# creanero/MKIDS_SDR

Hardware: AMD Instinct MI355X
Metric: ADC MSample/s/GPU at 1024 ch; achieved HBM GB/s vs roofline (higher is better)
Workload: dtype int16 in, fp32 DSP, int16 Fix16_13 trigger

## Files before the change

mkids_sdr_amd/csrc/k_trigger.hip:

```cpp
#include <algorithm>
#include <type_traits>

#include "mkid_plan.h"
#include "trig_common.h"

namespace mkid {

constexpr int kSpecThreads = 256;
constexpr int32_t kFullWarm = 100;

__device__ __forceinline__ int64_t seg_state(const TrigSpecArgs& a, int c, int s) { return (int64_t)c * a.nseg + s; }
__device__ __forceinline__ int64_t seg_begin(const TrigSpecArgs& a, int s) { return (int64_t)s * a.L; }
__device__ __forceinline__ int64_t seg_end(const TrigSpecArgs& a, int s) {
    return seg_begin(a, s) + a.L < a.J ? seg_begin(a, s) + a.L : a.J;
}
__device__ __forceinline__ int64_t slot_entry(const TrigSpecArgs& a, int c, int s) {
    return (int64_t)c * a.seg_stride + a.seg_base + s;
}
__device__ __forceinline__ TrigCfg trig_cfg(const TrigSpecArgs& a, int c) {
    return TrigCfg{a.thr[c], a.rearm[c], a.mode, a.alpha, a.kf, a.kq, a.base_thr, a.dead};
}

static_assert(plan::kSegL > kHoldOff + 1 && plan::kSvfLmin > kHoldOff + 1, "segments outlast the hold-off");

__device__ __forceinline__ int32_t raw_at(const TrigSpecArgs& a, int c, int64_t jj) {
    return jj >= 0 ? a.raw[jj * a.C + c] : (jj >= -kRawHist ? a.rhist[(jj + kRawHist) * a.C + c] : 0);
}

__device__ __attribute__((noinline)) uint64_t make_packet(int32_t c, EvInfo ev, int32_t f, int64_t jg) {
    return pack_wide(c, peakfit_i(ev.y1, ev.y2, f), ev.base, jg - 1);
}

struct Win {
    int32_t w[kFirTaps];
};

__device__ __forceinline__ void load_window(Win& win, const TrigSpecArgs& a, int c, int64_t j) {
    win.w[0] = 0;
#pragma unroll
    for (int i = 1; i < kFirTaps; ++i) win.w[i] = raw_at(a, c, j - kFirTaps + i);
}

__device__ __forceinline__ int32_t mf_at(const Win& win, const int32_t (&tap)[kFirTaps], int u) {
    int32_t acc = 0;
#pragma unroll
    for (int i = 0; i < kFirTaps; ++i) acc = __mul24(tap[i], win.w[(u - i + kFirTaps) % kFirTaps]) + acc;
    return mf_out(acc);
}

typedef short short2_t __attribute__((ext_vector_type(2)));
struct QWin {
    uint32_t q[kFirTaps];
    uint32_t last;
    uint32_t sel;
};

__device__ __forceinline__ uint32_t pack2(int32_t lo, int32_t hi) {
    return ((uint32_t)lo & 0xffffu) | ((uint32_t)hi << 16);
}

__device__ __forceinline__ short2_t as_s2(uint32_t v) { return __builtin_bit_cast(short2_t, v); }

__device__ __forceinline__ void load_tap_pairs(uint32_t (&tp)[kFirTaps / 2], const TrigSpecArgs& a, int c) {
#pragma unroll
    for (int m = 0; m < kFirTaps / 2; ++m) tp[m] = pack2(a.fir[c * kFirTaps + 2 * m], a.fir[c * kFirTaps + 2 * m + 1]);
}

__device__ __forceinline__ void load_qwin(QWin& w, const TrigSpecArgs& a, int c, int64_t j) {
    int32_t prev = 0;
#pragma unroll
    for (int i = 0; i < kFirTaps; ++i) {
        const int32_t r = raw_at(a, c, j - kFirTaps + i);
        w.q[i] = pack2(r, prev);
        prev = r;
    }
    w.last = pack2(prev, prev);
    w.sel = (c & 1) ? 0x07060302u : 0x05040100u;
}

struct Lim16 {
    int32_t lo, hi;
};
__device__ __forceinline__ Lim16 lim16() {
    Lim16 lim{-32768, 32767};
    asm volatile("" : "+v"(lim.lo), "+v"(lim.hi));
    return lim;
}
__device__ __forceinline__ int32_t mf_q(QWin& w, const uint32_t (&tp)[kFirTaps / 2], int u, uint32_t r,
                                        const Lim16& lim) {
    w.q[u] = __builtin_amdgcn_perm(w.last, r, w.sel);
    w.last = r;
    int32_t acc;
    asm("v_dot2_i32_i16 %0, %1, %2, 0" : "=v"(acc) : "v"(tp[0]), "v"(w.q[u]));
#pragma unroll
    for (int m = 1; m < kFirTaps / 2; ++m)
        acc = __builtin_amdgcn_sdot2(as_s2(tp[m]), as_s2(w.q[(u - 2 * m + 2 * kFirTaps) % kFirTaps]), acc, false);
    int32_t v;
    asm("v_med3_i32 %0, %1, %2, %3" : "=v"(v) : "v"(acc >> 11), "v"(lim.lo), "v"(lim.hi));
    return v;
}

__device__ __forceinline__ __amdgpu_buffer_rsrc_t raw_rsrc(const char* base) {
    return __builtin_amdgcn_make_buffer_rsrc(const_cast<char*>(base), (short)0, (int)0xffffffff, 0x00020000);
}

template <class F, class E>
__device__ __forceinline__ void run_groups(int32_t ngroups, const char* rbase, uint32_t& rrow, uint32_t lane,
                                           uint32_t row, F&& body, E&& half_end) {
    constexpr int H = kFirTaps / 2;
    const __amdgpu_buffer_rsrc_t rs = raw_rsrc(rbase);
    auto ld = [&](uint32_t off) { return (uint32_t)__builtin_amdgcn_raw_buffer_load_b32(rs, (int)lane, (int)off, 0); };
    auto uni = [](uint32_t v) { return (uint32_t)__builtin_amdgcn_readfirstlane((int)v); };
    uint32_t ra[H], rb[H];
    if (ngroups <= 0) return;
    rrow = uni(rrow);
#pragma unroll
    for (int u = 0; u < H; ++u) ra[u] = ld(rrow + (uint32_t)u * row);
    for (int32_t g = 0; g < ngroups; ++g) {
        const uint32_t cur = uni(rrow);
#pragma unroll
        for (int u = 0; u < H; ++u) rb[u] = ld(cur + (uint32_t)(H + u) * row);
#pragma unroll
        for (int u = 0; u < H; ++u) body(g, u, ra[u]);
        half_end(g, 0);
        const uint32_t nxt = uni(cur + (g + 1 < ngroups ? (uint32_t)kFirTaps * row : 0u));
#pragma unroll
        for (int u = 0; u < H; ++u) ra[u] = ld(nxt + (uint32_t)u * row);
#pragma unroll
        for (int u = 0; u < H; ++u) body(g, H + u, rb[u]);
        half_end(g, 1);
        rrow = cur + (uint32_t)kFirTaps * row;
    }
}
template <class F>
__device__ __forceinline__ void run_groups(int32_t ngroups, const char* rbase, uint32_t& rrow, uint32_t lane,
                                           uint32_t row, F&& body) {
    run_groups(ngroups, rbase, rrow, lane, row, body, [](int32_t, int) {});
}


template <int MODE, bool FAST = true>
struct Stepper {
    TrigState st;
    TrigCfg k;
    __device__ Stepper(const TrigState& s, const TrigCfg& kk) : st(s), k(kk) {}
    __device__ __forceinline__ bool step(int32_t f, EvInfo& ev) { return trig_update(st, f, k, ev); }
    __device__ __forceinline__ TrigState state() const { return st; }
};

template <int MODE>
struct Stepper<MODE, true> {
    FastState fs;
    FastCfg q;
    __device__ Stepper(const TrigState& s, const TrigCfg& k, int32_t f0) : fs(to_fast(s)), q(fast_cfg(k)) {
        if (!s.binit) fs.B = MODE == MKID_BASE_NONE ? 0 : f0;
    }
    __device__ __forceinline__ bool step(int32_t f, EvInfo& ev) { return trig_update_fast<MODE>(fs, f, q, ev); }
    __device__ __forceinline__ TrigState state() const { return from_fast(fs); }
};

template <>
struct Stepper<MKID_BASE_SVF, true> {
    FastSvf fs;
    FastCfg q;
    int32_t kf, kq;
    __device__ Stepper(const TrigState& s, const TrigCfg& k, int32_t f0)
        : fs(to_fast_svf(s)), q(fast_cfg(k)), kf(k.kf), kq(k.kq) {
        if (!s.binit) {
            fs.low = (int64_t)f0 * 65536;
            fs.band = 0;
        }
    }
    __device__ __forceinline__ bool step(int32_t f, EvInfo& ev) { return trig_update_svf(fs, f, q, kf, kq, ev); }
    __device__ __forceinline__ void step_base(int32_t f) { base_update_svf(fs, f, q, kf, kq); }
    __device__ __forceinline__ TrigState state() const { return from_fast_svf(fs); }
};

#ifndef MKID_TRIG_MINW
#define MKID_TRIG_MINW 4
#endif
__device__ __forceinline__ void set_progress_prio(int32_t done, int32_t ng) {
    const int32_t pc = done * 100;
    if (pc >= 95 * ng) __builtin_amdgcn_s_setprio(0);
    else if (pc >= 85 * ng) __builtin_amdgcn_s_setprio(1);
    else if (pc >= 70 * ng) __builtin_amdgcn_s_setprio(2);
}

template <int MODE>
__global__ __launch_bounds__(kSpecThreads, MKID_TRIG_MINW) void k_trig_spec(TrigSpecArgs a) {
    constexpr bool PRE = MODE == MKID_BASE_SVF;
    __builtin_amdgcn_s_setprio(3);
    const int64_t g = (int64_t)blockIdx.x * kSpecThreads + threadIdx.x;
    if (g >= (int64_t)a.C * a.nseg) return;
    const int C = a.C;
    const int c = (int)(g % C);
    const int s = (int)(g / C);
    uint32_t tp[kFirTaps / 2];
    if constexpr (!PRE) load_tap_pairs(tp, a, c);
    TrigCfg k = trig_cfg(a, c);
    k.mode = MODE;
    const int64_t seg0 = seg_begin(a, s), seg1 = seg_end(a, s);
    const int64_t jw = (s == 0 || seg0 <= a.W) ? 0 : seg0 - a.W;
    QWin win;
    if constexpr (!PRE) load_qwin(win, a, c, jw);
    const int64_t sc = slot_entry(a, c, s);
    uint64_t* slot = a.slots + sc * a.capseg;
    int32_t n = 0;
    const char* rbase = reinterpret_cast<const char*>((PRE ? a.filt : a.raw) +
                                                      (int64_t)__builtin_amdgcn_readfirstlane((int32_t)jw) * C);
    const uint32_t lane = (uint32_t)(c >> 1) * 4u;
    uint32_t rrow = 0;
    const __amdgpu_buffer_rsrc_t rs = raw_rsrc(rbase);
    auto rload = [&](uint32_t off) {
        return (uint32_t)__builtin_amdgcn_raw_buffer_load_b32(rs, (int)lane, __builtin_amdgcn_readfirstlane((int)off), 0);
    };
    const Lim16 lim = lim16();
    const uint32_t half = (uint32_t)(c & 1) * 16u;
    auto filt = [&](QWin& w, int u, uint32_t r) -> int32_t {
        if constexpr (PRE) return __builtin_amdgcn_sbfe((int32_t)r, half, 16);
        else return mf_q(w, tp, u, r, lim);
    };
    QWin w0 = win;
    const int32_t f0 = filt(w0, 0, rload(0));
    const TrigState st0 = jw == 0 ? a.st_in[c] : TrigState{0, 0, ST_REARM, 0, 0, 0, 0, 0, 0, 0};
    auto body = [&](auto& sp) {
        const int32_t wg = __builtin_amdgcn_readfirstlane((int32_t)(seg0 - jw) / kFirTaps);
        int32_t wbase = 0;
        if constexpr (MODE == MKID_BASE_SVF && std::is_same<std::decay_t<decltype(sp)>, Stepper<MODE, true>>::value) {
            wbase = (jw > 0 && wg > kFullWarm) ? wg - kFullWarm : 0;
            run_groups(wbase, rbase, rrow, lane, (uint32_t)(2 * C),
                       [&](int32_t, int u, uint32_t r) { sp.step_base(filt(win, u, r)); });
        }
        run_groups(wg - wbase, rbase, rrow, lane, (uint32_t)(2 * C),
                   [&](int32_t, int u, uint32_t r) {
                       EvInfo ev;
                       (void)sp.step(filt(win, u, r), ev);
                   });
        if (s > 0) a.s_spec[seg_state(a, c, s)] = sp.state();
        auto emit = [&](int64_t jg, int u, uint32_t r) {
            const int32_t f = filt(win, u, r);
            EvInfo ev;
            if (sp.step(f, ev)) {
                if (n < a.capseg) slot[n] = make_packet(c, ev, f, jg);
                ++n;
            }
        };
        const int32_t len = (int32_t)(seg1 - seg0);
        const int32_t full = len - len % kFirTaps;
        const int32_t ng = __builtin_amdgcn_readfirstlane(full / kFirTaps);
        run_groups(ng, rbase, rrow, lane, (uint32_t)(2 * C),
                   [&](int32_t gr, int u, uint32_t r) { emit(a.j0 + seg0 + gr * kFirTaps + u, u, r); },
                   [&](int32_t gr, int h) {
                       if (h == 1) set_progress_prio(gr + 1, ng);
                   });
        const int32_t left = len - full;
#pragma unroll
        for (int u = 0; u < kFirTaps; ++u)
            if (u < left) emit(a.j0 + seg0 + full + u, u, rload(rrow + (uint32_t)(2 * u * C)));
        a.s_end[seg_state(a, c, s)] = sp.state();
    };
    if (in_holdoff(st0)) {
        Stepper<MODE, false> sp(st0, k);
        body(sp);
    } else {
        Stepper<MODE> sp(st0, k, f0);
        body(sp);
    }
    a.counts[sc] = n;
}

__global__ __launch_bounds__(kSpecThreads) void k_mf_rows(TrigSpecArgs a, int32_t rows_per) {
    const int C = a.C;
    const int64_t g = (int64_t)blockIdx.x * kSpecThreads + threadIdx.x;
    const int c = (int)(g % C);
    const int64_t j0 = (g / C) * (int64_t)rows_per;
    if (j0 >= a.J) return;
    const int64_t j1 = j0 + rows_per < a.J ? j0 + rows_per : a.J;
    uint32_t tp[kFirTaps / 2];
    load_tap_pairs(tp, a, c);
    QWin win;
    load_qwin(win, a, c, j0);
    const int64_t jr = __builtin_amdgcn_readfirstlane((int32_t)j0);
    const char* rbase = reinterpret_cast<const char*>(a.raw + jr * C);
    const __amdgpu_buffer_rsrc_t out = raw_rsrc(reinterpret_cast<const char*>(a.filt + jr * C));
    const uint32_t lane = (uint32_t)(c >> 1) * 4u;
    const uint32_t lane16 = (uint32_t)c * 2u;
    const uint32_t row = (uint32_t)(2 * C);
    const Lim16 lim = lim16();
    auto put = [&](uint32_t roff, int u, uint32_t r) {
        __builtin_amdgcn_raw_buffer_store_b16((unsigned short)mf_q(win, tp, u, r, lim), out, (int)lane16,
                                              __builtin_amdgcn_readfirstlane((int)roff), 0);
    };
    uint32_t rrow = 0;
    const int32_t len = (int32_t)(j1 - j0);
    const int32_t ng = __builtin_amdgcn_readfirstlane(len / kFirTaps);
    run_groups(ng, rbase, rrow, lane, row,
               [&](int32_t gr, int u, uint32_t r) { put((uint32_t)(gr * kFirTaps + u) * row, u, r); });
    const int32_t left = len - ng * kFirTaps;
    const __amdgpu_buffer_rsrc_t rs = raw_rsrc(rbase);
#pragma unroll
    for (int u = 0; u < kFirTaps; ++u) {
        if (u < left) {
            const uint32_t ro = rrow + (uint32_t)u * row;
            put(ro, u, (uint32_t)__builtin_amdgcn_raw_buffer_load_b32(rs, (int)lane,
                                                                       __builtin_amdgcn_readfirstlane((int)ro), 0));
        }
    }
}

__device__ void splice_segment(const TrigSpecArgs& a, int c, int s, int32_t nt, int32_t ndrop, bool merged,
                               const uint64_t* scratch) {
    const int64_t sc = slot_entry(a, c, s);
    uint64_t* slot = a.slots + sc * a.capseg;
    const int32_t cnt = a.counts[sc] < a.capseg ? a.counts[sc] : a.capseg;
    int32_t total = nt;
    if (merged) {
        const int32_t keep = cnt - ndrop;
        if (nt < ndrop) {
            for (int32_t i = 0; i < keep; ++i) slot[nt + i] = slot[ndrop + i];
        } else if (nt > ndrop) {
            for (int32_t i = keep - 1; i >= 0; --i)
                if (nt + i < a.capseg) slot[nt + i] = slot[ndrop + i];
        }
        total = nt + (a.counts[sc] - ndrop);
    }
    for (int32_t i = 0; i < nt && i < a.capseg; ++i) slot[i] = scratch[i];
    a.counts[sc] = total;
}

__device__ bool rerun_segment(const TrigSpecArgs& a, int c, int s, const int32_t (&tap)[kFirTaps],
                              const TrigCfg& k, TrigState& T, const TrigState& S0) {
    const int64_t seg0 = seg_begin(a, s), seg1 = seg_end(a, s);
    uint64_t* scratch = a.scratch + (int64_t)c * a.capseg;
    TrigState tru = T, spc = S0;
    int32_t nt = 0, ndrop = 0;
    bool merged = false;
    Win win;
    load_window(win, a, c, seg0);
    const int16_t* rp = a.raw + seg0 * a.C + c;
    for (int64_t g = seg0; g < seg1 && !merged; g += kFirTaps) {
        const int64_t left = seg1 - g;
        int32_t r[kFirTaps];
#pragma unroll
        for (int u = 0; u < kFirTaps; ++u) r[u] = u < left ? rp[(int64_t)u * a.C] : 0;
        rp += (int64_t)kFirTaps * a.C;
#pragma unroll
        for (int u = 0; u < kFirTaps; ++u) {
            if (u >= left || merged) continue;
            const int64_t j = g + u;
            win.w[u] = r[u];
            const int32_t f = mf_at(win, tap, u);
            uint64_t pkt;
            if (trig_step(tru, f, k, c, a.j0 + j, &pkt)) {
                if (nt < a.capseg) scratch[nt] = pkt;
                ++nt;
            }
            uint64_t dummy;
            if (trig_step(spc, f, k, c, a.j0 + j, &dummy)) ++ndrop;
            merged = state_eq(tru, spc, a.mode);
        }
    }
    if (!merged) T = tru;
    splice_segment(a, c, s, nt, ndrop, merged, scratch);
    return merged;
}

__device__ __forceinline__ uint64_t readlane64(uint64_t v, int lane) {
    return ((uint64_t)(uint32_t)__builtin_amdgcn_readlane((int32_t)(v >> 32), lane) << 32) |
           (uint32_t)__builtin_amdgcn_readlane((int32_t)v, lane);
}

__device__ bool svf_walk(const TrigSpecArgs& a, int c, int s, const TrigCfg& k, const TrigState& T,
                         const TrigState& S0, int lane, uint64_t* out, int32_t& nt, int32_t& ndrop, TrigState& Tend) {
    const int64_t seg0 = seg_begin(a, s), seg1 = seg_end(a, s);
    const FastCfg q = fast_cfg(k);
    FastSvf st = to_fast_svf(lane == 0 ? T : S0);
    nt = 0;
    ndrop = 0;
    bool merged = false;
    const int16_t* fp = a.filt + c;
    __shared__ int32_t bsh[4][2][64];
    int32_t* bl = bsh[threadIdx.x >> 6][lane == 0 ? 0 : 1];
    int32_t fnext = seg0 + lane < seg1 ? (int32_t)fp[(seg0 + lane) * a.C] : 0;
    for (int64_t g = seg0; g < seg1 && !merged; g += 64) {
        const int32_t fl = fnext;
        asm volatile("" ::"v"(fl));
        const int left = __builtin_amdgcn_readfirstlane((int)(seg1 - g < 64 ? seg1 - g : 64));
        fnext = g + 64 + lane < seg1 ? (int32_t)fp[(g + 64 + lane) * a.C] : 0;
        const int32_t pf1 = __builtin_amdgcn_readlane(st.f1, 0), pf2 = __builtin_amdgcn_readlane(st.f2, 0);
        uint64_t em = 0;
        for (int i = 0; i < left; ++i) {
            const int32_t f = __builtin_amdgcn_readlane(fl, i);
            EvInfo ev;
            const bool e = trig_update_svf(st, f, q, a.kf, a.kq, ev);
            em |= (uint64_t)e << i;
            bl[i] = ev.base;
        }
        __builtin_amdgcn_wave_barrier();
        const uint64_t e0 = readlane64(em, 0), e1 = readlane64(em, 1);
        ndrop += __builtin_popcountll(e1);
        for (uint64_t m = e0; m; m &= m - 1) {
            const int i = __builtin_ctzll(m);
            const int32_t f = __builtin_amdgcn_readlane(fl, i);
            const int32_t y2 = i >= 1 ? __builtin_amdgcn_readlane(fl, i - 1) : pf1;
            const int32_t y1 = i >= 2 ? __builtin_amdgcn_readlane(fl, i - 2) : (i == 1 ? pf1 : pf2);
            if (lane == 0 && nt < a.capseg) out[nt] = make_packet(c, EvInfo{y1, y2, bsh[threadIdx.x >> 6][0][i]}, f, a.j0 + g + i);
            ++nt;
        }
        __builtin_amdgcn_wave_barrier();
        auto same = [&](int32_t v) { return __builtin_amdgcn_readlane(v, 0) == __builtin_amdgcn_readlane(v, 1); };
        merged = same((int32_t)st.low) && same((int32_t)(st.low >> 32)) && same((int32_t)st.band) &&
                 same((int32_t)(st.band >> 32)) && same(st.x) && same(st.f1) && same(st.f2);
    }
    if (!merged) {
        FastSvf t;
        t.low = (int64_t)readlane64((uint64_t)st.low, 0);
        t.band = (int64_t)readlane64((uint64_t)st.band, 0);
        t.x = __builtin_amdgcn_readlane(st.x, 0);
        t.f1 = __builtin_amdgcn_readlane(st.f1, 0);
        t.f2 = __builtin_amdgcn_readlane(st.f2, 0);
        Tend = from_fast_svf(t);
    }
    return merged;
}

__global__ __launch_bounds__(256) void k_trig_refix(TrigSpecArgs a) {
    const int C = a.C;
    const int64_t w = (int64_t)blockIdx.x * 4 + (threadIdx.x >> 6);
    const int lane = threadIdx.x & 63;
    if (w >= (int64_t)C * (a.nseg - 1)) return;
    const int c = (int)(w % C), s = (int)(w / C) + 1;
    const int64_t sc = slot_entry(a, c, s);
    RefixRes* res = a.refix + sc;
    const TrigState P = a.s_end[seg_state(a, c, s - 1)];
    const TrigState S0 = a.s_spec[seg_state(a, c, s)];
    int32_t status = RF_OK, nt = 0, ndrop = 0;
    TrigState Tend = P;
    if (!state_eq(P, S0, a.mode))
        status = svf_walk(a, c, s, trig_cfg(a, c), P, S0, lane, a.refix_pk + sc * a.capseg, nt, ndrop, Tend)
                     ? RF_MERGED
                     : RF_UNMERGED;
    if (lane == 0) {
        res->status = status;
        res->nt = nt;
        res->ndrop = ndrop;
        res->T = Tend;
    }
}

__global__ __launch_bounds__(64) void k_trig_fix(TrigSpecArgs a) {
    extern __shared__ uint64_t okbits[];
    const int c = blockIdx.x;
    const int lane = threadIdx.x;
    const int nwords = (a.nseg + 63) / 64;
    for (int wd0 = 0; wd0 < nwords; wd0 += 4) {
        bool ok[4];
#pragma unroll
        for (int i = 0; i < 4; ++i) {
            const int s = (wd0 + i) * 64 + lane;
            const bool valid = s >= 1 && s < a.nseg;
            const int64_t ie = seg_state(a, c, valid ? s - 1 : 0), ip = seg_state(a, c, valid ? s : 0);
            const TrigState e = a.s_end[ie];
            const TrigState p = a.s_spec[ip];
            ok[i] = !valid || state_eq_nb(e, p, a.mode);
        }
#pragma unroll
        for (int i = 0; i < 4; ++i) {
            const uint64_t b = __ballot(ok[i]);
            if (lane == 0 && wd0 + i < nwords) okbits[wd0 + i] = b;
        }
    }
    __syncthreads();
    if (lane != 0) return;
    int32_t tap[kFirTaps];
#pragma unroll
    for (int i = 0; i < kFirTaps; ++i) tap[i] = a.fir[c * kFirTaps + i];
    const TrigCfg k = trig_cfg(a, c);
    int32_t reruns = 0;
    TrigState T{};
    bool override_ = false;
    int s = 1;
    while (s < a.nseg) {
        if (!override_) {
            int wd = s >> 6;
            uint64_t fail = ~okbits[wd] & (~0ull << (s & 63));
            while (!fail && ++wd < nwords) fail = ~okbits[wd];
            if (!fail) break;
            s = wd * 64 + __builtin_ctzll(fail);
            if (s >= a.nseg) break;
            T = a.s_end[seg_state(a, c, s - 1)];
        } else if (state_eq(T, a.s_spec[seg_state(a, c, s)], a.mode)) {
            override_ = false;
            ++s;
            continue;
        }
        ++reruns;
        const TrigState S0 = a.s_spec[seg_state(a, c, s)];
        override_ = !rerun_segment(a, c, s, tap, k, T, S0);
        ++s;
    }
    a.st_out[c] = override_ ? T : a.s_end[seg_state(a, c, a.nseg - 1)];
    if (a.reruns) a.reruns[c] = reruns;
}

__global__ __launch_bounds__(64) void k_trig_fix_svf(TrigSpecArgs a) {
    const int c = blockIdx.x;
    const int lane = threadIdx.x;
    const TrigCfg k = trig_cfg(a, c);
    uint64_t* scratch = a.scratch + (int64_t)c * a.capseg;
    int32_t reruns = 0;
    bool truth = true;
    TrigState T{};
    for (int s = 1; s < a.nseg; ++s) {
        if (truth) {
            const int64_t sc = slot_entry(a, c, s);
            const RefixRes* r = a.refix + sc;
            const int32_t st = r->status;
            if (st == RF_OK) continue;
            ++reruns;
            if (lane == 0) splice_segment(a, c, s, r->nt, r->ndrop, st == RF_MERGED, a.refix_pk + sc * a.capseg);
            if (st == RF_UNMERGED) {
                T = r->T;
                truth = false;
            }
            continue;
        }
        const TrigState S0 = a.s_spec[seg_state(a, c, s)];
        if (state_eq(T, S0, a.mode)) {
            truth = true;
            continue;
        }
        ++reruns;
        int32_t nt, ndrop;
        TrigState Tend = T;
        truth = svf_walk(a, c, s, k, T, S0, lane, scratch, nt, ndrop, Tend);
        if (lane == 0) splice_segment(a, c, s, nt, ndrop, truth, scratch);
        if (!truth) T = Tend;
        __syncthreads();
    }
    if (lane != 0) return;
    a.st_out[c] = truth ? a.s_end[seg_state(a, c, a.nseg - 1)] : T;
    if (a.reruns) a.reruns[c] = reruns;
}

int64_t trigger_wave_slots(int device) {
    int ncu = 0, nb = 0;
    if (hipDeviceGetAttribute(&ncu, hipDeviceAttributeMultiprocessorCount, device) != hipSuccess || ncu <= 0)
        ncu = 256;
    if (hipOccupancyMaxActiveBlocksPerMultiprocessor(&nb, k_trig_spec<MKID_BASE_EMA>, kSpecThreads, 0) != hipSuccess ||
        nb <= 0)
        nb = 1;
    return (int64_t)ncu * nb * (kSpecThreads / 64);
}

hipError_t launch_trigger(const TrigSpecArgs& a, hipStream_t s) {
    const int64_t threads = (int64_t)a.C * a.nseg;
    const dim3 grid((unsigned)((threads + kSpecThreads - 1) / kSpecThreads));
    hipError_t e;
    if (a.mode == MKID_BASE_SVF) {
        if (!a.filt || !a.refix || !a.refix_pk) return hipErrorInvalidValue;
        const int64_t nt = std::max<int64_t>(1, (int64_t)3072 * 64 / a.C);
        int64_t rp = std::max<int64_t>(520, (a.J + nt - 1) / nt);
        rp = (rp + kFirTaps - 1) / kFirTaps * kFirTaps;
        const int64_t mthreads = (int64_t)a.C * ((a.J + rp - 1) / rp);
        hipLaunchKernelGGL(k_mf_rows, dim3((unsigned)((mthreads + kSpecThreads - 1) / kSpecThreads)),
                           dim3(kSpecThreads), 0, s, a, (int32_t)rp);
        if ((e = hipGetLastError()) != hipSuccess) return e;
        hipLaunchKernelGGL(k_trig_spec<MKID_BASE_SVF>, grid, dim3(kSpecThreads), 0, s, a);
        if ((e = hipGetLastError()) != hipSuccess) return e;
        if (a.nseg > 1) {
            const int64_t waves = (int64_t)a.C * (a.nseg - 1);
            hipLaunchKernelGGL(k_trig_refix, dim3((unsigned)((waves + 3) / 4)), dim3(256), 0, s, a);
            if ((e = hipGetLastError()) != hipSuccess) return e;
        }
        hipLaunchKernelGGL(k_trig_fix_svf, dim3(a.C), dim3(64), 0, s, a);
        return hipGetLastError();
    }
    if (a.mode == MKID_BASE_EMA)
        hipLaunchKernelGGL(k_trig_spec<MKID_BASE_EMA>, grid, dim3(kSpecThreads), 0, s, a);
    else
        hipLaunchKernelGGL(k_trig_spec<MKID_BASE_NONE>, grid, dim3(kSpecThreads), 0, s, a);
    if ((e = hipGetLastError()) != hipSuccess) return e;
    const size_t lds = (size_t)((a.nseg + 63) / 64) * 8;
    hipLaunchKernelGGL(k_trig_fix, dim3(a.C), dim3(64), lds, s, a);
    return hipGetLastError();
}

}
```

mkids_sdr_amd/csrc/trig_common.h:

```cpp
#pragma once
#include "mkid_internal.h"

namespace mkid {

enum { ST_ARMED = 0, ST_PULSE = 1, ST_DEAD = 2, ST_REARM = 3 };

struct TrigCfg {
    int32_t thr, rearm, mode, alpha, kf, kq, base_thr, dead;
};

__device__ __forceinline__ int32_t tclamp16(int32_t v) { return v < -32768 ? -32768 : (v > 32767 ? 32767 : v); }
__device__ __forceinline__ int32_t tclampi(int32_t v, int32_t lo, int32_t hi) { return v < lo ? lo : (v > hi ? hi : v); }

__device__ __forceinline__ int64_t peakfit_i(int64_t y1, int64_t y2, int64_t y3) {
    const int64_t den = y3 + y1 - 2 * y2;
    if (den == 0) return y2;
    const int64_t d = y3 - y1;
    return y2 - (d * d) / (8 * den);
}

__device__ __forceinline__ uint64_t pack_wide(int32_t ch, int64_t peak, int32_t base, int64_t j) {
    const uint64_t pk = (uint64_t)tclampi((int32_t)((peak >> 4) + 2048), 0, 4095);
    const uint64_t bs = (uint64_t)tclampi((base >> 4) + 2048, 0, 4095);
    return ((uint64_t)(ch & 0xFFF) << MKID_PKT_CH_SHIFT) | (pk << MKID_PKT_PEAK_SHIFT) |
           (bs << MKID_PKT_BASE_SHIFT) | ((uint64_t)j & MKID_PKT_TS_MASK);
}

__device__ __forceinline__ int32_t mf_out(int32_t acc) { return tclamp16(acc >> 11); }

struct EvInfo {
    int32_t y1, y2, base;
};

__device__ __attribute__((noinline)) uint64_t make_packet(int32_t c, EvInfo ev, int32_t f, int64_t jg);

__device__ __forceinline__ bool trig_update(TrigState& s, int32_t f, const TrigCfg& k, EvInfo& ev) {
    if (!s.binit && s.st != ST_DEAD) {
        s.B = (k.mode == MKID_BASE_NONE) ? 0 : f;
        s.low = (int64_t)f * 65536;
        s.band = 0;
        s.binit = 1;
    }
    const int32_t base_prev = (k.mode == MKID_BASE_SVF) ? (int32_t)(s.low >> 16) : s.B;
    const int32_t e = f - base_prev;
    const bool gate = (k.base_thr <= 0) || (e < k.base_thr && e > -k.base_thr);
    if (k.mode == MKID_BASE_EMA && s.binit) {
        s.B += gate ? ((k.alpha * e) >> 9) : 0;
    } else if (k.mode == MKID_BASE_SVF && gate && s.binit) {
        const int64_t high = ((int64_t)f * 65536) - s.low - (((int64_t)k.kq * s.band) >> 16);
        s.band += ((int64_t)k.kf * high) >> 16;
        s.low += ((int64_t)k.kf * s.band) >> 16;
    }
    const bool armed = s.st == ST_ARMED, pulse = s.st == ST_PULSE, dead = s.st == ST_DEAD;
    const bool rearm = s.st == ST_REARM;
    const bool emit = pulse && (f > s.f1);
    const int32_t cnt1 = s.cnt - 1;
    const bool to_pulse = armed && (e < k.thr);
    const bool to_rearm = dead && (cnt1 <= 0);
    const bool to_armed = rearm && (e >= k.rearm);
    ev = EvInfo{s.f2, s.f1, base_prev};
    s.cnt = emit ? k.dead : (dead ? cnt1 : s.cnt);
    s.st = to_pulse ? ST_PULSE : (emit ? ST_DEAD : (to_rearm ? ST_REARM : (to_armed ? ST_ARMED : s.st)));
    s.f2 = s.f1;
    s.f1 = f;
    return emit;
}

__device__ __forceinline__ bool in_holdoff(const TrigState& s) { return !s.binit && s.st == ST_DEAD; }

struct FastState {
    int32_t B, x, f1, f2;
};
struct FastCfg {
    int32_t thr, rearm, alpha, dx;
    uint32_t goff, glim;
};

__device__ __forceinline__ FastCfg fast_cfg(const TrigCfg& k) {
    FastCfg q{k.thr, k.rearm, k.alpha, k.dead > 1 ? k.dead : 1, 0x80000000u, 0xffffffffu};
    if (k.base_thr > 0) {
        q.goff = (uint32_t)k.base_thr - 1u;
        q.glim = 2u * (uint32_t)k.base_thr - 1u;
    }
    return q;
}

__device__ __forceinline__ FastState to_fast(const TrigState& s) {
    const int32_t x = s.st == ST_ARMED ? -1 : (s.st == ST_PULSE ? -2 : (s.st == ST_REARM ? 0 : (s.cnt > 1 ? s.cnt : 1)));
    return FastState{s.B, x, s.f1, s.f2};
}

__device__ __forceinline__ TrigState from_fast(const FastState& f) {
    const int32_t st = f.x == -1 ? ST_ARMED : (f.x == -2 ? ST_PULSE : (f.x == 0 ? ST_REARM : ST_DEAD));
    return TrigState{f.B, 1, st, f.x > 0 ? f.x : 0, f.f1, f.f2, 0, 0, 0, 0};
}

__device__ __forceinline__ bool code_step(int32_t& x, int32_t e, int32_t f, int32_t f1, const FastCfg& k) {
    const bool emit = (x == -2) & (f > f1);
    int32_t xn = e < (x == 0 ? k.rearm : k.thr) ? 2 * x : -1;
    xn = x == -2 ? (f > f1 ? k.dx : -2) : xn;
    xn = x > 0 ? x - 1 : xn;
    x = xn;
    return emit;
}

template <int MODE>
__device__ __forceinline__ bool trig_update_fast(FastState& s, int32_t f, const FastCfg& k, EvInfo& ev) {
    const int32_t e = f - s.B;
    ev = EvInfo{s.f2, s.f1, s.B};
    if (MODE == MKID_BASE_EMA) {
        const int32_t gate = -(int32_t)((uint32_t)e + k.goff < k.glim);
        s.B += (__mul24(k.alpha, e) >> 9) & gate;
    }
    const bool emit = code_step(s.x, e, f, s.f1, k);
    s.f2 = s.f1;
    s.f1 = f;
    return emit;
}

struct FastSvf {
    int64_t low, band;
    int32_t x, f1, f2;
};

__device__ __forceinline__ FastSvf to_fast_svf(const TrigState& s) {
    const FastState f = to_fast(s);
    return FastSvf{s.low, s.band, f.x, f.f1, f.f2};
}

__device__ __forceinline__ TrigState from_fast_svf(const FastSvf& f) {
    TrigState t = from_fast(FastState{0, f.x, f.f1, f.f2});
    t.low = f.low;
    t.band = f.band;
    return t;
}

__device__ __forceinline__ int64_t mul_u32_i64(uint32_t a, int64_t b) {
    const uint64_t lo = (uint64_t)a * (uint32_t)b;
    const uint32_t hi = a * (uint32_t)((uint64_t)b >> 32);
    return (int64_t)(lo + ((uint64_t)hi << 32));
}

__device__ __forceinline__ void svf_update(FastSvf& s, int32_t f, int32_t e, const FastCfg& k, int32_t kf, int32_t kq) {
    const bool gate = (uint32_t)e + k.goff < k.glim;
    const int64_t high = ((int64_t)f * 65536) - s.low - (mul_u32_i64((uint32_t)kq, s.band) >> 16);
    const int64_t band = s.band + (mul_u32_i64((uint32_t)kf, high) >> 16);
    const int64_t low = s.low + (mul_u32_i64((uint32_t)kf, band) >> 16);
    s.band = gate ? band : s.band;
    s.low = gate ? low : s.low;
}

__device__ __forceinline__ void base_update_svf(FastSvf& s, int32_t f, const FastCfg& k, int32_t kf, int32_t kq) {
    svf_update(s, f, f - (int32_t)(s.low >> 16), k, kf, kq);
    s.f2 = s.f1;
    s.f1 = f;
}

__device__ __forceinline__ bool trig_update_svf(FastSvf& s, int32_t f, const FastCfg& k, int32_t kf, int32_t kq,
                                                EvInfo& ev) {
    const int32_t base = (int32_t)(s.low >> 16);
    const int32_t e = f - base;
    ev = EvInfo{s.f2, s.f1, base};
    svf_update(s, f, e, k, kf, kq);
    const bool emit = code_step(s.x, e, f, s.f1, k);
    s.f2 = s.f1;
    s.f1 = f;
    return emit;
}

__device__ __forceinline__ bool trig_step(TrigState& s, int32_t f, const TrigCfg& k, int32_t c,
                                          int64_t jg, uint64_t* pkt) {
    EvInfo ev;
    if (!trig_update(s, f, k, ev)) return false;
    *pkt = make_packet(c, ev, f, jg);
    return true;
}

__device__ __forceinline__ bool state_eq_nb(const TrigState& a, const TrigState& b, int mode) {
    bool eq = (a.binit == b.binit) & (a.st == b.st) & (a.f1 == b.f1) & (a.f2 == b.f2);
    eq &= (a.st != ST_DEAD) | (a.cnt == b.cnt);
    const bool base = mode == MKID_BASE_EMA ? a.B == b.B
                                            : (mode == MKID_BASE_SVF ? (a.low == b.low) & (a.band == b.band) : true);
    return eq & (!a.binit | base);
}

__device__ __forceinline__ bool state_eq(const TrigState& a, const TrigState& b, int mode) {
    if (a.binit != b.binit || a.st != b.st || a.f1 != b.f1 || a.f2 != b.f2) return false;
    if (a.st == ST_DEAD && a.cnt != b.cnt) return false;
    if (!a.binit) return true;
    if (mode == MKID_BASE_EMA) return a.B == b.B;
    if (mode == MKID_BASE_SVF) return a.low == b.low && a.band == b.band;
    return true;
}

}
```

Baseline: 228,300.

## Track trigger state as wave-wide ballot masks and use 32-bit peak fit

The per-lane trigger state code (armed, pulse, rearm, dead countdown) is replaced by 64-bit wave ballot masks held in scalar registers. A running sample index plus a per-lane deadline replaces the decrementing dead counter, and an inline asm move sets the deadline only in lanes that emit. The aim is to move the state-machine logic onto cheap scalar mask operations and cut per-sample vector ALU work. Separately, the 64-bit integer peak-fit division becomes a 32-bit quotient computed through double-precision division, avoiding a slow 64-bit integer divide. The risks are that the mask path assumes a fully converged wave64, and that state conversion forces binit to 1 and zeroes the SVF fields.

```diff
diff --git a/mkids_sdr_amd/csrc/k_trigger.hip b/mkids_sdr_amd/csrc/k_trigger.hip
--- a/mkids_sdr_amd/csrc/k_trigger.hip
+++ b/mkids_sdr_amd/csrc/k_trigger.hip
@@ -28,7 +28,7 @@
 }
 
 __device__ __attribute__((noinline)) uint64_t make_packet(int32_t c, EvInfo ev, int32_t f, int64_t jg) {
-    return pack_wide(c, peakfit_i(ev.y1, ev.y2, f), ev.base, jg - 1);
+    return pack_wide(c, peakfit32(ev.y1, ev.y2, f), ev.base, jg - 1);
 }
 
 struct Win {
@@ -150,13 +150,13 @@
 
 template <int MODE>
 struct Stepper<MODE, true> {
-    FastState fs;
+    MaskState ms;
     FastCfg q;
-    __device__ Stepper(const TrigState& s, const TrigCfg& k, int32_t f0) : fs(to_fast(s)), q(fast_cfg(k)) {
-        if (!s.binit) fs.B = MODE == MKID_BASE_NONE ? 0 : f0;
-    }
-    __device__ __forceinline__ bool step(int32_t f, EvInfo& ev) { return trig_update_fast<MODE>(fs, f, q, ev); }
-    __device__ __forceinline__ TrigState state() const { return from_fast(fs); }
+    __device__ Stepper(const TrigState& s, const TrigCfg& k, int32_t f0) : ms(to_mask(s)), q(fast_cfg(k)) {
+        if (!s.binit) ms.B = MODE == MKID_BASE_NONE ? 0 : f0;
+    }
+    __device__ __forceinline__ bool step(int32_t f, EvInfo& ev) { return trig_update_mask<MODE>(ms, f, q, ev); }
+    __device__ __forceinline__ TrigState state() const { return from_mask(ms); }
 };
 
 template <>
diff --git a/mkids_sdr_amd/csrc/peakfit32.h b/mkids_sdr_amd/csrc/peakfit32.h
--- /dev/null
+++ b/mkids_sdr_amd/csrc/peakfit32.h
@@ -0,0 +1,30 @@
+#pragma once
+#include <stdint.h>
+#if !defined(__HIP__) && !defined(__CUDACC__)
+#include <assert.h>
+#endif
+
+#if defined(__HIP__) || defined(__CUDACC__)
+#define MKID_PF_HD __attribute__((host)) __attribute__((device))
+#else
+#define MKID_PF_HD
+#endif
+
+namespace mkid {
+
+MKID_PF_HD inline int32_t peakfit32_quot(int32_t d, int32_t den) {
+#if !defined(__HIP__) && !defined(__CUDACC__)
+    assert(d >= -65535 && d <= 65535 && den >= -131070 && den <= 131070);
+#endif
+    const uint32_t n = (uint32_t)d * (uint32_t)d;
+    const uint32_t m = 8u * (uint32_t)(den < 0 ? -den : den);
+    const int32_t q = den == 0 ? 0 : (int32_t)(uint32_t)((double)n / (double)m);
+    return den < 0 ? -q : q;
+}
+
+MKID_PF_HD inline int32_t peakfit32(int32_t y1, int32_t y2, int32_t y3) {
+    const int32_t den = y3 + y1 - 2 * y2;
+    return den == 0 ? y2 : y2 - peakfit32_quot(y3 - y1, den);
+}
+
+}
diff --git a/mkids_sdr_amd/csrc/trig_common.h b/mkids_sdr_amd/csrc/trig_common.h
--- a/mkids_sdr_amd/csrc/trig_common.h
+++ b/mkids_sdr_amd/csrc/trig_common.h
@@ -1,5 +1,6 @@
 #pragma once
 #include "mkid_internal.h"
+#include "peakfit32.h"
 
 namespace mkid {
 
@@ -12,15 +13,8 @@
 __device__ __forceinline__ int32_t tclamp16(int32_t v) { return v < -32768 ? -32768 : (v > 32767 ? 32767 : v); }
 __device__ __forceinline__ int32_t tclampi(int32_t v, int32_t lo, int32_t hi) { return v < lo ? lo : (v > hi ? hi : v); }
 
-__device__ __forceinline__ int64_t peakfit_i(int64_t y1, int64_t y2, int64_t y3) {
-    const int64_t den = y3 + y1 - 2 * y2;
-    if (den == 0) return y2;
-    const int64_t d = y3 - y1;
-    return y2 - (d * d) / (8 * den);
-}
-
-__device__ __forceinline__ uint64_t pack_wide(int32_t ch, int64_t peak, int32_t base, int64_t j) {
-    const uint64_t pk = (uint64_t)tclampi((int32_t)((peak >> 4) + 2048), 0, 4095);
+__device__ __forceinline__ uint64_t pack_wide(int32_t ch, int32_t peak, int32_t base, int64_t j) {
+    const uint64_t pk = (uint64_t)tclampi((peak >> 4) + 2048, 0, 4095);
     const uint64_t bs = (uint64_t)tclampi((base >> 4) + 2048, 0, 4095);
     return ((uint64_t)(ch & 0xFFF) << MKID_PKT_CH_SHIFT) | (pk << MKID_PKT_PEAK_SHIFT) |
            (bs << MKID_PKT_BASE_SHIFT) | ((uint64_t)j & MKID_PKT_TS_MASK);
@@ -104,18 +98,46 @@
     return emit;
 }
 
+struct MaskState {
+    int32_t B, tl, f1, f2;
+    uint64_t armed, pulse, rearm;
+    int32_t i;
+};
+
+__device__ __forceinline__ uint64_t lanes_where(bool p) { return __builtin_amdgcn_ballot_w64(p); }
+__device__ __forceinline__ bool in_lanes(uint64_t m) { return __builtin_amdgcn_inverse_ballot_w64(m); }
+
+__device__ __forceinline__ MaskState to_mask(const TrigState& s) {
+    return MaskState{s.B, (s.cnt > 1 ? s.cnt : 1) - 1, s.f1, s.f2, lanes_where(s.st == ST_ARMED),
+                     lanes_where(s.st == ST_PULSE), lanes_where(s.st == ST_REARM), 0};
+}
+
+__device__ __forceinline__ TrigState from_mask(const MaskState& m) {
+    const int32_t st = in_lanes(m.armed) ? ST_ARMED : (in_lanes(m.pulse) ? ST_PULSE : (in_lanes(m.rearm) ? ST_REARM : ST_DEAD));
+    return TrigState{m.B, 1, st, st == ST_DEAD ? m.tl - m.i + 1 : 0, m.f1, m.f2, 0, 0, 0, 0};
+}
+
 template <int MODE>
-__device__ __forceinline__ bool trig_update_fast(FastState& s, int32_t f, const FastCfg& k, EvInfo& ev) {
+__device__ __forceinline__ bool trig_update_mask(MaskState& s, int32_t f, const FastCfg& k, EvInfo& ev) {
     const int32_t e = f - s.B;
     ev = EvInfo{s.f2, s.f1, s.B};
     if (MODE == MKID_BASE_EMA) {
         const int32_t gate = -(int32_t)((uint32_t)e + k.goff < k.glim);
         s.B += (__mul24(k.alpha, e) >> 9) & gate;
     }
-    const bool emit = code_step(s.x, e, f, s.f1, k);
-    s.f2 = s.f1;
-    s.f1 = f;
-    return emit;
+    const uint64_t ct = lanes_where(e < k.thr), cr = lanes_where(e < k.rearm), cf = lanes_where(f > s.f1);
+    const uint64_t last = lanes_where(s.tl == s.i);
+    const uint64_t dead = ~(s.armed | s.pulse | s.rearm);
+    const uint64_t emit = s.pulse & cf;
+    if (in_lanes(emit)) asm volatile("v_mov_b32 %0, %1" : "+v"(s.tl) : "s"(s.i + k.dx));
+    const uint64_t armed = (s.armed & ~ct) | (s.rearm & ~cr);
+    s.pulse = (s.pulse & ~cf) | (s.armed & ct);
+    s.rearm = (s.rearm & cr) | (dead & last);
+    s.armed = armed;
+    s.f2 = s.f1;
+    s.f1 = f;
+    s.i += 1;
+    return in_lanes(emit);
 }
 
 struct FastSvf {
```

Result: no change. 229,400 (median of 6 runs) (+0.5%).
